# clintpgeorge/LDAGroupedGibbsSampler

Measured on AMD Instinct MI355X. Metric: M tokens sampled/sec (whole node) per Gibbs sweep at K=100, higher is better.
Workload: dtype f64

## Files before the change

ldagroupedgibbssampler_amd/csrc/ggs_api.hip:

```cpp
#include <hip/hip_runtime.h>

#include <algorithm>
#include <cmath>
#include <cstdio>
#include <cstdlib>
#include <cstring>
#include <new>
#include <string>
#include <vector>

#include "ggs_kernels.hpp"
#include "ggs_z_sliced.hpp"
#include "ggs_z_stream.hpp"
#include "ggs_exact_sum.hpp"
#include "ggs_z_pcgs.hpp"
#include "ggs_z_pcgs_wave.hpp"
#include "ggs_z_collapsed.hpp"
#include "ggs_phi_poisson.hpp"
#include "ggs_alias.hpp"
#include "ggs_z_spalias.hpp"
#include "ggs_z_polyaurn_sparse.hpp"
#include "ggs_phi_vs.hpp"
#include "ggs_z_lightpc.hpp"
#include "ggs_z_lightcollapsed.hpp"
// ... 97 lines not shown
  bool have_corpus = false, have_phi = false, in_sweep = false;
  int32_t num_cus = 0;
  LaunchPlan plan;
  const LaunchPlan::ZCfg *cfg = nullptr;
  int32_t *d_chunk_doc1 = nullptr;
  double margin_scale = 1.0;
  double margin_scale32 = 1.0;

  hipStream_t stream = nullptr;
  int64_t *d_doc_ptr = nullptr, *d_chunk_start = nullptr;
  int32_t *d_tok = nullptr, *d_z = nullptr, *d_chunk_doc = nullptr, *d_chunk_len = nullptr;
  int32_t *d_ct_tok = nullptr, *d_ct_idx = nullptr, *d_ct_ip = nullptr, *d_c_docs = nullptr, *d_hot_words = nullptr;
  int64_t Cs = 0, Cc = 0;
  int32_t *d_order = nullptr;
  int64_t pcgs_order_len = 0;
  bool pcgs_wave = false;
  KernelLaunch pcgs_z;
  int64_t pcgs_items = 0;
  int32_t pa_L = 0;
  double pa_t00 = 0;
  double *d_pa_table = nullptr;
  unsigned long long *d_pa_acc = nullptr;
  bool alias_stale = true;
  double *d_alias_ps = nullptr, *d_alias_tn = nullptr;
  int32_t *d_alias_a = nullptr;
  int32_t sp_cap = 0;
  bool have_priors = false;
  int32_t pr_pitch = 0;
  std::vector<uint32_t> pr_mask;
  uint32_t *d_pr_mask = nullptr;
  double *d_pr_sum_phi = nullptr;
  double *d_pr_pref = nullptr, *d_pr_fn = nullptr;
  double alpha_sum = 0;
  unsigned long long *d_mh = nullptr;
  int32_t *d_tpt = nullptr;
  uint16_t *d_nzw = nullptr;
  int32_t *d_nw = nullptr;
  unsigned long long *d_ps_stats = nullptr;
  double vs_pi = 0.5;
  bool vs_global = false;
  int32_t vs_W = 0, vs_pitch = 0;
  uint32_t *d_vs_cz = nullptr, *d_vs_pz = nullptr, *d_vs_und = nullptr;
  uint32_t *d_vs_mask = nullptr;
  int32_t *d_vs_work = nullptr, *d_vs_s_end = nullptr, *d_vs_rounds = nullptr;
  unsigned long long *d_vs_zero = nullptr;
  enum class VsLists { empty, drawn, nonzero } vs_lists = VsLists::empty;
  bool vs_drawn = false;
  uint64_t *d_lcg = nullptr;
  bool lcg_ready = false;
  int32_t num_hot = 0;
  int32_t *d_perm = nullptr, *d_inv_perm = nullptr, *d_zw = nullptr, *d_seg_word = nullptr, *d_seg_begin = nullptr;
  double *d_theta_next = nullptr;
  hipStream_t side = nullptr;
  hipStream_t side_hot = nullptr;
  hipEvent_t ev_hot_fork = nullptr, ev_hot_join = nullptr;
  bool theta_main = true, chain_on_side = false, theta_main_always = false;
  bool whole_sweep = false;
  hipEvent_t hot_fork_from = nullptr;
  hipEvent_t ev_chain_done = nullptr;
  bool z_split = true, z_split_tried = false;
  int32_t warm_tiers = 0, num_warm = 0, warm_rows_max = 0;
  int64_t Cw = 0, warm_chunks_max = 0;
  int32_t *d_wt_pack = nullptr, *d_w_docs = nullptr, *d_warm_words = nullptr;
  int32_t *d_ht_pack = nullptr, *d_h_docs = nullptr;
  int64_t *d_warm_meta = nullptr;
  bool overlap_theta = true;
// ... 615 lines not shown
  return GGS_OK;
}

int launch_phi(ggs_handle *h, bool initial, bool accumulate_mean, Events *E = nullptr) {
  int rc;
  if (h->xg) {
    if ((rc = phi_step_a(h)) || (rc = phi_step_a_clear(h))) return rc;
    if (E) HIP_TRY(h, hipEventRecord(E->x[0], h->stream));
    if ((rc = phi_step_b1(h, initial)) || (rc = phi_step_g0(h)) || (rc = phi_step_b2(h, initial))) return rc;
    if (E) HIP_TRY(h, hipEventRecord(E->x[1], h->stream));
    if ((rc = phi_join_halves(h)) || (rc = phi_step_g1(h))) return rc;
    if (E) HIP_TRY(h, hipEventRecord(E->x[2], h->stream));
    if ((rc = phi_step_c(h, initial, accumulate_mean))) return rc;
    return launch_alias_build(h);
  }
  if (conditional_phi(h, initial) && (rc = launch_sum_phi(h))) return rc;
  if ((rc = launch_phi_slice(h, initial, h->d_n_wk, h->K, h->K, 0, h->d_phiT, h->Kp, h->d_mag, h->d_tot, h->d_n_k, accumulate_mean ? h->d_phi_mean : nullptr)))
    return rc;
  h->n_k_valid = true;
  h->have_phi = true;
  if (h->scheme == Scheme::nzvsspalias) { h->vs_lists = initial ? ggs_handle::VsLists::empty : ggs_handle::VsLists::drawn; if (initial) h->vs_drawn = false; }
  if (h->have_priors && initial && (rc = phi_apply_priors(h))) return rc;
  return launch_alias_build(h);
}

int launch_theta(ggs_handle *h, hipStream_t stream, double *dst, int32_t iteration, int64_t d0 = 0, int64_t d1 = -1, int32_t lds = 0, int32_t docs_per_block = 0) {
  if (d1 < 0) d1 = h->D;
  if (d1 <= d0) return GGS_OK;
  if (docs_per_block <= 0) docs_per_block = h->cfg->theta_docs;
  ThetaParams tp{};
  tp.doc_ptr = h->d_doc_ptr + d0; tp.z = h->d_z; tp.alpha = h->d_alpha; tp.theta = dst + (size_t)d0 * h->K; tp.status = h->d_status;
  tp.num_docs = d1 - d0; tp.doc_base = h->doc_base + d0; tp.seed = h->seed; tp.iteration = (uint32_t)iteration;
  tp.K = h->K; tp.docs_per_block = docs_per_block; tp.queue_cap = std::min(kGammaQueue, h->gamma_queue_cap);
  const int64_t grid = (d1 - d0 + docs_per_block - 1) / docs_per_block;
  void *args[] = {&tp};
  HIP_TRY(h, hipLaunchKernel(h->plan.theta.fn, dim3((unsigned)grid), dim3(kThetaBlock), args, (size_t)(lds ? lds : h->cfg->theta_lds), stream));
  return GGS_OK;
}

#define GGS_KMAX_SWITCH(KERNEL)                                                                                                     \
  switch ((K + 7) / 8) {                                                                                                            \
    case 1: return reinterpret_cast<const void *>(KERNEL<8>);      case 2: return reinterpret_cast<const void *>(KERNEL<16>);       \
    case 3: return reinterpret_cast<const void *>(KERNEL<24>);     case 4: return reinterpret_cast<const void *>(KERNEL<32>);       \
    case 5: return reinterpret_cast<const void *>(KERNEL<40>);     case 6: return reinterpret_cast<const void *>(KERNEL<48>);       \
    case 7: return reinterpret_cast<const void *>(KERNEL<56>);     case 8: return reinterpret_cast<const void *>(KERNEL<64>);       \
    case 9: return reinterpret_cast<const void *>(KERNEL<72>);     case 10: return reinterpret_cast<const void *>(KERNEL<80>);      \
    case 11: return reinterpret_cast<const void *>(KERNEL<88>);    case 12: return reinterpret_cast<const void *>(KERNEL<96>);      \
    case 13: return reinterpret_cast<const void *>(KERNEL<104>);   case 14: return reinterpret_cast<const void *>(KERNEL<112>);     \
    case 15: return reinterpret_cast<const void *>(KERNEL<120>);   case 16: return reinterpret_cast<const void *>(KERNEL<128>);     \
    case 17: return reinterpret_cast<const void *>(KERNEL<136>);   case 18: return reinterpret_cast<const void *>(KERNEL<144>);     \
    case 19: return reinterpret_cast<const void *>(KERNEL<152>);   case 20: return reinterpret_cast<const void *>(KERNEL<160>);     \
    case 21: return reinterpret_cast<const void *>(KERNEL<168>);   case 22: return reinterpret_cast<const void *>(KERNEL<176>);     \
    case 23: return reinterpret_cast<const void *>(KERNEL<184>);   default: return reinterpret_cast<const void *>(KERNEL<192>);     \
  }
const void *sliced_kernel_for(int K) { GGS_KMAX_SWITCH(z_sliced_kernel) }
const void *sliced32_kernel_for(int K) { GGS_KMAX_SWITCH(z_sliced32_kernel) }

const void *hot_kernel_for(int K) { GGS_KMAX_SWITCH(z_hot_kernel) }
const void *warm_kernel_for(int K) { GGS_KMAX_SWITCH(z_warm_kernel) }
const void *pcgs_kernel_for(int K) { GGS_KMAX_SWITCH(pcgs_sliced_kernel) }
const void *polyaurn_kernel_for(int K) { GGS_KMAX_SWITCH(polyaurn_sliced_kernel) }
const void *collapsed_kernel_for(int K) {
  switch ((K + 7) / 8) {
#define GGS_CK(N) case N: return reinterpret_cast<const void *>(pcgs_sliced_kernel<8 * N, true>);
    GGS_CK(1) GGS_CK(2) GGS_CK(3) GGS_CK(4) GGS_CK(5) GGS_CK(6) GGS_CK(7) GGS_CK(8) GGS_CK(9) GGS_CK(10) GGS_CK(11) GGS_CK(12)
    GGS_CK(13) GGS_CK(14) GGS_CK(15) GGS_CK(16) GGS_CK(17) GGS_CK(18) GGS_CK(19) GGS_CK(20) GGS_CK(21) GGS_CK(22) GGS_CK(23)
// ... 54 lines not shown
      pl.z.lds = two_pass ? z_stream_lds_bytes(K) : z_stream1_lds_bytes(K, group, pl.two_rows, regck);
      if (pl.z.lds > kMaxLdsBytes) return GGS_ERR_UNSUPPORTED;
    } else if (sliced) {
      pl.f32 = !kn.phi64.is(1);
      pl.Kp32 = round_up(K, kSlice32Topics);
      pl.ring_base = sliced_ring_base(K); pl.wave_lds = sliced_wave_lds(K); pl.hot_pitch = table_row_pitch(K);
      pl.hot_wave_lds = hot_wave_lds(K); pl.warm_wave_lds = warm_wave_lds(K);
      if (kn.split.set) { pl.split = kn.split.v != 0; pl.split_forced = kn.split.v == 2; }
      pl.hot_cap = pl.split ? table_rows_beside_cold(K, pl.hot_wave_lds) : table_rows_fused(K);
      if (kn.hot.set) pl.hot_cap = std::max(0, std::min(pl.hot_cap, kn.hot.v));
      pl.cold = {pl.f32 ? sliced32_kernel_for(K) : sliced_kernel_for(K), kSlicedWaves * 64, sliced_cold_lds(K), 1};
      pl.hot = {hot_kernel_for(K), kSlicedWaves * 64, table_lds(K, pl.hot_wave_lds, 0), 1};
      pl.warm = {warm_kernel_for(K), kSlicedWaves * 64, table_lds(K, pl.warm_wave_lds, 0), 1};
      pl.warm_docs = warm_docs_for(sliced_kmax(K));
      pl.warm_cap = table_rows_beside_cold(K, pl.warm_wave_lds);
      if (pl.warm_cap < 16) pl.warm_cap = 0;
      if (kn.warm.set) pl.warm_tiers_max = std::max(0, std::min(kWarmMaxTiers, kn.warm.v));
      if (kn.warm_rows.set) pl.warm_cap = std::max(0, std::min(pl.warm_cap, kn.warm_rows.v));
      if (kn.warm_fill.set) pl.warm_min_fill_pct = std::max(1, std::min(100, kn.warm_fill.v));
      if (kn.warm_cpw.set) pl.warm_min_chunks_per_wave = std::max(0, kn.warm_cpw.v);
    } else {
      int T = z_tile_rows_in(kMaxLdsBytes / 6 / kLdsGranule * kLdsGranule, Kp, pitch16);
      if (kn.tile.set) T = kn.tile.v;
      pl.tile_tokens = std::max(8, std::min(64, T));
      pl.z.fn = tile_kernel_for(K);
      pl.z.lds = z_tile_lds_bytes(Kp, pitch16, pl.tile_tokens);
      if (pl.z.lds > kMaxLdsBytes) return GGS_ERR_UNSUPPORTED;
    }
    if (!sliced) {
      pl.z.per_cu = lds_workgroups_per_cu(pl.z.lds, 8);
      if (kn.wpc.set) pl.z.per_cu = std::max(1, kn.wpc.v);
    }
  }
  int B = 64;
  while (B > 1 && theta_lds_bytes(K, B) > 32 * 1024) B >>= 1;
  if (theta_lds_bytes(K, B) > kMaxLdsBytes) return GGS_ERR_UNSUPPORTED;
  pl.theta.fn = reinterpret_cast<const void *>(theta_kernel<kThetaBlock>); pl.theta.block = kThetaBlock;
  const int theta_quarter = (kMaxLdsBytes - 24 * 1024) / 4;
  pl.cfg_plain = {1, pl.z.per_cu, B, std::max(theta_lds_bytes(K, B), theta_quarter), 0};
  pl.theta_docs_main = kn.theta_b.set ? std::max(1, std::min(B, kn.theta_b.v)) : std::min(B, 16);
  pl.theta_lds_main = std::max(theta_lds_bytes(K, pl.theta_docs_main), (kMaxLdsBytes - 24 * 1024) / (kn.theta_wgs.set ? std::max(1, kn.theta_wgs.v) : 5));
  pl.cfg_parts = pl.cfg_plain;
  if (scheme == Scheme::ggs) {
    pl.parts_forced = kn.zparts.set;
    int parts = kn.zparts.set ? std::max(1, std::min(8, kn.zparts.v)) : pl.kernel == 2 ? 8 : 1;
    if (parts > 1 && pl.kernel == 2) {
      const int kBeside = kn.beside.set ? std::max(1, kn.beside.v) : 4;
      int Bt = 64;
      while (Bt > 1 && theta_lds_bytes(K, Bt) > 10 * 1024) Bt >>= 1;
      const int t_lds = theta_lds_bytes(K, Bt), z_alloc = lds_alloc_of(pl.z.lds);
      const int zw = std::min(pl.z.per_cu, (kMaxLdsBytes - kLdsGranule - kBeside * lds_alloc_of(t_lds)) / z_alloc);
      if (t_lds <= 12 * 1024 && zw >= 2)
        pl.cfg_parts = {parts, zw, Bt, std::max(t_lds, theta_quarter), std::max(t_lds, (kMaxLdsBytes - kLdsGranule - zw * z_alloc) / kBeside / kLdsGranule * kLdsGranule)};
      else
        parts = 1;
    }
    pl.cfg_parts.parts = parts;
    return GGS_OK;
  }

  const bool collapsed = scheme == Scheme::collapsed, polyaurn = scheme == Scheme::polyaurn;
  if (K <= kPcgsWaveMaxTopics) {
    const int nb = pcgs_wave_blocks(Kp);
    pl.wave.fn = pcgs_wave_kernel_for(nb, collapsed, polyaurn);
    pl.wave.lds = pcgs_wave_lds_bytes(nb);
    int by_regs = 0;
    if (hipOccupancyMaxActiveBlocksPerMultiprocessor(&by_regs, pl.wave.fn, 64, (size_t)pl.wave.lds) != hipSuccess || by_regs < 1) by_regs = 1;
    pl.wave.per_cu = lds_workgroups_per_cu(pl.wave.lds, std::min(by_regs, 32));
  }
  pl.wave_forced = kn.pcgs_wave.set ? kn.pcgs_wave.v != 0 : K > (collapsed ? kCollapsedWaveFromTopics : polyaurn ? kPolyaurnWaveFromTopics : kPcgsWaveFromTopics);
  if (pl.wave_forced && !pl.wave.fn) return GGS_ERR_UNSUPPORTED;
  const bool lane_sliced = K <= kSlicedMaxTopics && !(kn.pcgs_stream.set && kn.pcgs_stream.v != 0);
  pl.lane.lds = lane_sliced ? pcgs_sliced_lds_bytes(K) : pcgs_z_lds_bytes(K);
  if (pl.lane.lds > kMaxLdsBytes && !pl.wave_forced) return GGS_ERR_UNSUPPORTED;
  pl.lane.per_cu = lds_workgroups_per_cu(pl.lane.lds, 8);
  if (!pl.wave_forced) pl.lane.fn = pcgs_lane_kernel_for(K, lane_sliced, collapsed, polyaurn);
  if (collapsed) pl.serial.fn = reinterpret_cast<const void *>(collapsed_serial_kernel);
  if (has_alias(scheme)) {
    pl.alias_wpb = alias_words_per_block(K);
    pl.alias = {reinterpret_cast<const void *>(alias_build_kernel), 64, (int)alias_lds_bytes(K, pl.alias_wpb), 0};
    pl.alias.per_cu = lds_workgroups_per_cu(pl.alias.lds, 16);
  }
  if (scheme == Scheme::spalias) pl.spalias.fn = reinterpret_cast<const void *>(spalias_wave_kernel);
  if (scheme == Scheme::polyaurn_sparse) {
    pl.wordlist = {reinterpret_cast<const void *>(word_list_build_kernel), kWordListBlock, 0, 8};
// ... 500 lines not shown

}

extern "C" {

int ggs_abi_version(void) { return GGS_ABI_VERSION; }

const char *ggs_last_error(const ggs_handle *h) { return h ? h->err.c_str() : "null handle"; }

int ggs_create(const ggs_config *cfg, ggs_handle **out) {
  if (!cfg || !out) return GGS_ERR_BAD_ARG;
  *out = nullptr;
  if (cfg->struct_size != (int32_t)sizeof(ggs_config)) return GGS_ERR_BAD_ARG;
  if (cfg->num_topics <= 0 || cfg->num_types <= 0 || !(cfg->beta > 0)) return GGS_ERR_BAD_ARG;
  Scheme scheme = Scheme::ggs; int32_t poisson_L = 0;
  if (const int rc = scheme_of(cfg, scheme, poisson_L)) return rc;
  int ndev = 0;
  if (hipGetDeviceCount(&ndev) != hipSuccess || ndev <= 0 || cfg->device_id < 0 || cfg->device_id >= ndev) return GGS_ERR_HIP;
  ggs_handle *h = new (std::nothrow) ggs_handle();
  if (!h) return GGS_ERR_HIP;
  const Knobs kn;
  h->K = cfg->num_topics; h->V = cfg->num_types; h->device = cfg->device_id;
  h->Ks = h->Ksm = h->K; h->k0 = 0;
  h->Kp = (h->K + 1) & ~1;
  h->pitch16 = (h->Kp / 2) | 1;
  h->beta = cfg->beta; h->seed = cfg->seed; h->flags = cfg->flags;
  h->scheme = scheme; h->pa_L = poisson_L;
  h->phi_burn_in = cfg->phi_burn_in; h->phi_thin = cfg->phi_mean_thin > 0 ? cfg->phi_mean_thin : 1;
  h->alpha.assign(h->K, cfg->alpha_scalar);
  if (cfg->alpha) std::copy(cfg->alpha, cfg->alpha + h->K, h->alpha.begin());
  for (double a : h->alpha)
    if (!(a > 0)) { delete h; return GGS_ERR_BAD_ARG; }
  for (double a : h->alpha) h->alpha_sum = h->alpha_sum + a;
  if (kn.margin.set) { h->margin_scale = std::max(1.0, kn.margin.f); h->margin_scale32 = std::max(0.0, kn.margin.f); }
  if (kn.chain.set) h->exact_sum = kn.chain.v == 0;
  if (kn.guided.set) h->sum_guided = kn.guided.v != 0;
  if (kn.no_overlap.set) h->overlap_theta = kn.no_overlap.v == 0;
  if (kn.theta_main.set) { h->theta_main = kn.theta_main.v != 0; h->theta_main_always = kn.theta_main.v == 2; }
  if (kn.gamma_queue.set) h->gamma_queue_cap = std::max(0, kn.gamma_queue.v);
  h->sum_nseg = (h->V + kSumSegRows - 1) / kSumSegRows;

  int rc = GGS_OK;
  auto bail = [&](int code) { ggs_destroy(h); return code; };
  if (hipSetDevice(h->device) != hipSuccess) return bail(GGS_ERR_HIP);
  {
    hipDeviceProp_t prop;
    if (hipGetDeviceProperties(&prop, h->device) != hipSuccess) return bail(GGS_ERR_HIP);
    h->num_cus = prop.multiProcessorCount > 0 ? prop.multiProcessorCount : 256;
    if (kn.num_cus.set) h->num_cus = std::max(1, std::min(h->num_cus, kn.num_cus.v));
  }
  if ((rc = plan_launches(h->K, h->V, h->scheme, kn, h->plan))) return bail(rc);
  h->cfg = &h->plan.cfg_parts;
  h->z_split = h->plan.split;
  if (pcgs_family(h->scheme)) h->pcgs_z = pcgs_entry(h->plan, h->scheme, h->plan.wave_forced);
  for (const KernelLaunch *l : h->plan.all())
    if (l->fn && hipFuncSetAttribute(l->fn, hipFuncAttributeMaxDynamicSharedMemorySize, kMaxLdsBytes) != hipSuccess) return bail(GGS_ERR_HIP);
  for (const void *f : {reinterpret_cast<const void *>(ll_docs_kernel), reinterpret_cast<const void *>(lp_docs_kernel)})
    if (hipFuncSetAttribute(f, hipFuncAttributeMaxDynamicSharedMemorySize, kMaxLdsBytes) != hipSuccess) return bail(GGS_ERR_HIP);
  const bool with_phi = h->scheme != Scheme::lightcollapsed;
  const size_t kv = (size_t)h->K * h->V, phi_elems = (size_t)h->V * h->Kp + kPhiTailPadBytes / 8;
  if ((rc = dev_alloc(h, &h->d_alpha, h->K)) || (with_phi && (rc = dev_alloc(h, &h->d_phiT, phi_elems))) ||
      (rc = dev_alloc(h, &h->d_mag, h->K)) || (rc = dev_alloc(h, &h->d_tot, h->K)) || (rc = dev_alloc(h, &h->d_n_wk, kv)) ||
      (rc = dev_alloc(h, &h->d_n_k, h->K)) || (rc = dev_alloc(h, &h->d_status, 4)))
    return bail(rc);
  if ((h->flags & GGS_FLAG_SAVE_PHI_MEAN) && (rc = dev_alloc(h, &h->d_phi_mean, kv))) return bail(rc);
  if (h->plan.sliced() && h->plan.f32) {
// ... 1366 lines not shown
```

ldagroupedgibbssampler_amd/csrc/ggs_device_math.hpp:

```cpp
#pragma once
#include <hip/hip_runtime.h>
#include <stdint.h>

#include "../../include/ggs_hip.h"
#include "ggs_layout.hpp"

namespace ggs {

struct U4 { uint32_t x, y, z, w; };

__device__ __forceinline__ U4 philox4x32_10(uint32_t c0, uint32_t c1, uint32_t c2, uint32_t c3,
                                            uint32_t k0, uint32_t k1) {
  constexpr uint32_t M0 = 0xD2511F53u, M1 = 0xCD9E8D57u, W0 = 0x9E3779B9u, W1 = 0xBB67AE85u;
#pragma unroll
  for (int r = 0; r < 10; ++r) {
    const uint64_t p0 = (uint64_t)M0 * c0, p1 = (uint64_t)M1 * c2;
    const uint32_t hi0 = (uint32_t)(p0 >> 32), lo0 = (uint32_t)p0;
    const uint32_t hi1 = (uint32_t)(p1 >> 32), lo1 = (uint32_t)p1;
    const uint32_t n0 = hi1 ^ c1 ^ k0, n2 = hi0 ^ c3 ^ k1;
    c0 = n0; c1 = lo1; c2 = n2; c3 = lo0;
    k0 += W0; k1 += W1;
  }
  return U4{c0, c1, c2, c3};
}
// ... 256 lines not shown
      : k0((uint32_t)seed), k1((uint32_t)(seed >> 32)), c0((uint32_t)elem), c1((uint32_t)(elem >> 32)),
        c2base(purpose << 24), c3(iter), pos(0), cached(-1), d0(0), d1(0), next_gauss(0),
        have_gauss(false), exhausted(false) {}

  __device__ __forceinline__ double next_double() {
    const uint32_t blk = pos >> 1;
    if (blk >= (uint32_t)GGS_MAX_BLOCKS) { exhausted = true; return 0.5; }
    if ((int32_t)blk != cached) {
      const U4 o = philox4x32_10(c0, c1, c2base | blk, c3, k0, k1);
      d0 = u53(o.x, o.y);
      d1 = u53(o.z, o.w);
      cached = (int32_t)blk;
    }
    const double d = (pos & 1u) ? d1 : d0;
    ++pos;
    return d;
  }
  __device__ __forceinline__ double next_gaussian() {
    if (have_gauss) { have_gauss = false; return next_gauss; }
    double v1, v2, s;
    do {
      v1 = 2 * next_double() - 1;
      v2 = 2 * next_double() - 1;
      s = v1 * v1 + v2 * v2;
      if (exhausted) return 0.0;
    } while (s >= 1 || s == 0);
    const double multiplier = sqrt(-2 * strict_log(s) / s);
    next_gauss = v2 * multiplier;
    have_gauss = true;
    return v1 * multiplier;
  }
};

__device__ __forceinline__ double prgamma(DrawStream &r, double alpha) {
  const double d = alpha - (1.0 / 3.0);
  const double c = 1.0 / sqrt(9.0 * d);
  for (;;) {
    double x, v;
    do {
      x = r.next_gaussian();
      v = 1.0 + c * x;
      if (r.exhausted) return __builtin_nan("");
    } while (v <= 0.0);
    v = v * v * v;
    const double u = r.next_double();
    if (u < (1.0 - 0.0331 * (x * x) * (x * x))) return d * v;
    if (strict_log(u) < (0.5 * x * x + d * (1.0 - v + strict_log(v)))) return d * v;
    if (r.exhausted) return __builtin_nan("");
  }
}
__device__ __forceinline__ double rgamma(DrawStream &r, double alpha) {
  const bool boost = alpha < 1;
  const double u = r.next_double();
  const double g = prgamma(r, boost ? 1 + alpha : alpha);
  return boost ? g * strict_pow(u, 1.0 / alpha) : g;
}

__device__ __forceinline__ bool rgamma_first_try(uint64_t seed, uint32_t iter, uint32_t purpose, uint64_t elem, double alpha, double &g) {
  const uint32_t k0 = (uint32_t)seed, k1 = (uint32_t)(seed >> 32), c0 = (uint32_t)elem, c1 = (uint32_t)(elem >> 32), c2 = purpose << 24;
  const U4 b0 = philox4x32_10(c0, c1, c2, iter, k0, k1), b1 = philox4x32_10(c0, c1, c2 | 1u, iter, k0, k1),
           b2 = philox4x32_10(c0, c1, c2 | 2u, iter, k0, k1);
  const double u0 = u53(b0.x, b0.y);
  const double a1 = 2 * u53(b0.z, b0.w) - 1, a2 = 2 * u53(b1.x, b1.y) - 1, sa = a1 * a1 + a2 * a2;
  const double w = u53(b1.z, b1.w);
  const double e1 = 2 * w - 1, e2 = 2 * u53(b2.x, b2.y) - 1, sb = e1 * e1 + e2 * e2;
  const bool ok_a = !(sa >= 1 || sa == 0), ok_b = !(sb >= 1 || sb == 0);
  if (!(ok_a || ok_b)) return false;
  const double v1 = ok_a ? a1 : e1, s = ok_a ? sa : sb;
  const double u = ok_a ? w : u53(b2.z, b2.w);
  const double multiplier = sqrt(-2 * strict_log(s) / s);
  const double x = v1 * multiplier;
  const bool boost = alpha < 1;
  const double shape = boost ? 1 + alpha : alpha;
  const double d = shape - (1.0 / 3.0);
  const double c = 1.0 / sqrt(9.0 * d);
  double v = 1.0 + c * x;
  if (!(v > 0.0)) return false;
  v = v * v * v;
  if (!(u < (1.0 - 0.0331 * (x * x) * (x * x)))) return false;
  const double r = d * v;
  g = boost ? r * strict_pow(u0, 1.0 / alpha) : r;
  return true;
}

}
```

ldagroupedgibbssampler_amd/csrc/ggs_kernels.hpp:

```cpp
#pragma once
#include "ggs_device_math.hpp"
#include "ggs_exact_sum.hpp"

namespace ggs {

constexpr double kJavaMinValue = 4.9e-324;

__device__ __forceinline__ uint32_t udiv_magic(uint32_t d) { return d > 1 ? (uint32_t)((0x100000000ull + d - 1) / d) : 0u; }
__device__ __forceinline__ int udiv_small(int x, uint32_t m) { return m ? (int)__umulhi((uint32_t)x, m) : x; }

enum StatusBits : uint32_t {
  ST_NEGATIVE_COUNT = 1u << 0,
  ST_INVALID_TOPIC = 1u << 1,
  ST_RNG_EXHAUSTED = 1u << 2,
  ST_BAD_SHAPE = 1u << 3,
  ST_INVARIANT = 1u << 4,
};

struct ThetaParams {
  const int64_t *doc_ptr;
  const int32_t *z;
  const double *alpha;
  double *theta;
  uint32_t *status;
  int64_t num_docs, doc_base;
  uint64_t seed;
  uint32_t iteration;
  int32_t K, docs_per_block;
  int32_t queue_cap;
};

constexpr int kGammaQueue = 768;
constexpr int kThetaQueueBytes = 8 + 2 * kGammaQueue;
constexpr int theta_lds_bytes(const int K, const int b) { return (int)((size_t)K * (b | 1) * 8 + (size_t)b * 20 + kThetaQueueBytes); }

template <int BLOCK>
__global__ __launch_bounds__(BLOCK) void theta_kernel(ThetaParams p) {
  extern __shared__ __align__(16) unsigned char smem[];
  const int K = p.K, B = p.docs_per_block, BP = B | 1;
  double *gam = reinterpret_cast<double *>(smem);
  int32_t *hist = reinterpret_cast<int32_t *>(smem);
  double *mag = gam + (size_t)K * BP;
  double *tot = mag + B;
  int32_t *len = reinterpret_cast<int32_t *>(tot + B);
  int32_t *qn = len + B;
  uint16_t *queue = reinterpret_cast<uint16_t *>(qn + 2);

  const int tid = threadIdx.x;
  const int64_t d0 = (int64_t)blockIdx.x * B;
  const int nb = (int)min((int64_t)B, p.num_docs - d0);

  for (int i = tid; i < K * BP; i += BLOCK) hist[2 * i] = 0;
  if (tid == 0) *qn = 0;
  __syncthreads();

  constexpr int NW = BLOCK / 64;
  const int wave = tid >> 6, lane = tid & 63;
  for (int b = wave; b < nb; b += NW) {
    const int64_t beg = p.doc_ptr[d0 + b], end = p.doc_ptr[d0 + b + 1];
    if (lane == 0) len[b] = (int32_t)(end - beg);
    for (int64_t i = beg + lane; i < end; i += 64) atomicAdd(&hist[2 * (p.z[i] * BP + b)], 1);
  }
  __syncthreads();

  if (tid < nb && len[tid] > 0) {
    double m = 0;
    for (int k = 0; k < K; ++k) m += (double)hist[2 * (k * BP + tid)] + p.alpha[k];
    mag[tid] = m;
  }
  __syncthreads();

  auto shape_of = [&](int k, int b) {
    const double pk = (double)hist[2 * (k * BP + b)] + p.alpha[k];
    const double m = mag[b];
    return (pk / m) * m;
  };
  auto draw_general = [&](int k, int b, double shape) {
    DrawStream rs(p.seed, p.iteration, GGS_PURPOSE_THETA, (uint64_t)(p.doc_base + d0 + b) * (uint64_t)K + (uint64_t)k);
    const double g = rgamma(rs, shape);
    if (rs.exhausted) atomicOr(p.status, ST_RNG_EXHAUSTED);
    return g;
  };
  const uint32_t m_nb = udiv_magic((uint32_t)max(nb, 1)), m_K = udiv_magic((uint32_t)K);
  for (int i = tid; i < nb * K; i += BLOCK) {
    const int k = udiv_small(i, m_nb), b = i - k * nb;
    if (len[b] == 0) continue;
    const double shape = shape_of(k, b);
    double g;
    if (shape > 0) {
      if (!rgamma_first_try(p.seed, p.iteration, GGS_PURPOSE_THETA, (uint64_t)(p.doc_base + d0 + b) * (uint64_t)K + (uint64_t)k, shape, g)) {
        const int slot = atomicAdd(qn, 1);
        if (slot < p.queue_cap) { queue[slot] = (uint16_t)i; continue; }
        g = draw_general(k, b, shape);
      }
    } else {
      g = __builtin_nan("");
      atomicOr(p.status, ST_BAD_SHAPE);
    }
    gam[k * BP + b] = g;
  }
  __syncthreads();
  for (int q = tid, m = min(*qn, p.queue_cap); q < m; q += BLOCK) {
    const int i = queue[q], k = udiv_small(i, m_nb), b = i - k * nb;
    gam[k * BP + b] = draw_general(k, b, shape_of(k, b));
  }
  __syncthreads();

  if (tid < nb && len[tid] > 0) {
    double s = 0;
    for (int k = 0; k < K; ++k) s += gam[k * BP + tid];
    tot[tid] = s;
  }
  __syncthreads();

  for (int i = tid; i < nb * K; i += BLOCK) {
    const int b = udiv_small(i, m_K), k = i - b * K;
    if (len[b] == 0) continue;
    double v = gam[k * BP + b];
    const double s = tot[b];
    if (s != 0) {
      v = v / s;
      if (v <= 0) v = kJavaMinValue;
    }
// ... 214 lines not shown

struct PhiGammaParams {
  const int32_t *n_wk;
  const double *mag;
  double *phiT;
  uint32_t *status;
  uint64_t seed;
  uint32_t iteration, purpose;
  int32_t K, Kp, V;
  int32_t cnt_pitch, k0;
  double beta;
  double prior_pm;
  int32_t initial;
  int32_t kc, ncg;
  int32_t seg_begin, seg_end;
  int32_t queue_cap;
  int32_t prio;
  const double *guess;
  double *fn;
  const uint32_t *zero_mask;
  int32_t mask_pitch;
  int32_t undrawn_negative;
};
constexpr double kConditionalMinGamma = 0.0001;

constexpr int kPhiCols = 6, kPhiQueue = 128;

enum PhiDraw { kDrawPlain, kDrawPriors, kDrawVS };
template <int MODE>
__device__ __forceinline__ void phi_gamma_body(const PhiGammaParams &p) {
  constexpr bool PRIORS = MODE == kDrawPriors, MASKED = MODE != kDrawPlain;
  if (p.prio) __builtin_amdgcn_s_setprio(1);
  __shared__ uint16_t queue[kPhiQueue];
  __shared__ int32_t qn;
  __shared__ double acc_lo[kPhiCols], acc_hi[kPhiCols];
  __shared__ int32_t e_los[kPhiCols], aheads[kPhiCols], flag_s[kPhiCols];
  const int lane = threadIdx.x;
  const int64_t tiles = (int64_t)(p.seg_end - p.seg_begin) * p.ncg;
  auto shape_of = [&](int v, int k) {
    const int32_t cnt = p.n_wk[(size_t)v * p.cnt_pitch + k];
    if (p.initial) return (cnt == 0) ? p.prior_pm : p.prior_pm + (double)cnt;
    const double pk = p.beta + (double)cnt;
    if constexpr (MODE == kDrawVS) return pk;
    const double m = p.mag[k];
    return (pk / m) * m;
  };
  auto draw_general = [&](int v, int k, double shape) {
    DrawStream rs(p.seed, p.iteration, p.purpose, (uint64_t)(p.k0 + k) * (uint64_t)p.V + (uint64_t)v);
    const double g = rgamma(rs, shape);
    if (rs.exhausted) atomicOr(p.status, ST_RNG_EXHAUSTED);
    return g;
  };
  const uint32_t m_ncg = udiv_magic((uint32_t)p.ncg);
  for (int64_t tile = blockIdx.x; tile < tiles; tile += gridDim.x) {
    const int si = udiv_small((int)tile, m_ncg), cg = (int)tile - si * p.ncg;
    const int seg = p.seg_begin + si, v0 = seg * 64, kb = cg * p.kc, kw = min(p.kc, p.K - kb);
    const int rows = min(64, p.V - v0), n = rows * kw;
    const uint32_t m_kw = udiv_magic((uint32_t)kw);
    __syncthreads();
    if (lane < kw) {
      SegCand c{kSegNoGuess, true};
      if (p.guess) c = seg_candidates(p.guess[(size_t)seg * p.K + kb + lane], p.guess[(size_t)(seg + 1) * p.K + kb + lane]);
      e_los[lane] = c.e_lo; aheads[lane] = c.ahead ? 1 : 0; acc_lo[lane] = 0; acc_hi[lane] = 0; flag_s[lane] = 0;
    }
    if (lane == 0) qn = 0;
    __syncthreads();
    auto emit = [&](int v, int c, double g) {
      if constexpr (PRIORS) { if (g <= 0) g = kConditionalMinGamma; }
      p.phiT[(size_t)v * p.Kp + kb + c] = g;
      const int e_lo = e_los[c];
      if (e_lo == kSegNoGuess) return;
      double q_lo, q_hi;
      int fl;
      seg_quantise(g, e_lo, q_lo, q_hi, fl);
      seg_accumulate(&acc_lo[c], &acc_hi[c], &flag_s[c], q_lo, q_hi, fl);
    };
#pragma unroll 1
    for (int j = lane; j < n; j += 64) {
      const int dv = udiv_small(j, m_kw), v = v0 + dv, c = j - dv * kw, k = kb + c;
      if constexpr (MASKED) {
        const int kg = p.k0 + k;
        if ((p.zero_mask[(size_t)v * p.mask_pitch + (kg >> 5)] >> (kg & 31)) & 1u) {
          p.phiT[(size_t)v * p.Kp + k] = (MODE == kDrawVS && p.undrawn_negative) ? -0.0 : 0.0;
          continue;
        }
      }
      const double shape = shape_of(v, k);
      double g;
      if (shape > 0) {
        if (!rgamma_first_try(p.seed, p.iteration, p.purpose, (uint64_t)(p.k0 + k) * (uint64_t)p.V + (uint64_t)v, shape, g)) {
          const int slot = atomicAdd(&qn, 1);
          if (slot < p.queue_cap) { queue[slot] = (uint16_t)j; continue; }
          g = draw_general(v, k, shape);
        }
      } else {
        g = __builtin_nan("");
        atomicOr(p.status, ST_BAD_SHAPE);
      }
      emit(v, c, g);
    }
    __syncthreads();
    for (int q = lane, m = min(qn, p.queue_cap); q < m; q += 64) {
      const int j = queue[q], dv = udiv_small(j, m_kw), v = v0 + dv, c = j - dv * kw;
      emit(v, c, draw_general(v, kb + c, shape_of(v, kb + c)));
    }
    __syncthreads();
    if (p.guess && lane < kw)
      seg_compose(SegCand{e_los[lane], aheads[lane] != 0}, acc_lo[lane], acc_hi[lane], flag_s[lane], 0.0, p.fn + ((size_t)seg * p.K + kb + lane) * 4);
  }
}
template <bool PRIORS>
__global__ __launch_bounds__(64) void phi_gamma_kernel(PhiGammaParams p) { phi_gamma_body<PRIORS ? kDrawPriors : kDrawPlain>(p); }
__global__ __launch_bounds__(64) void phi_gamma_vs_kernel(PhiGammaParams p) { phi_gamma_body<kDrawVS>(p); }

__device__ __forceinline__ float phi32_of(const double x) { return (x >= 0.0 && x <= 1.0) ? (float)x : __builtin_nanf(""); }

enum PhiNorm { kPhiDirichlet, kPhiPolyaurn, kPhiConditional, kPhiVS };
template <int MODE>
__device__ __forceinline__ void phi_normalise_body(double *phiT, const double *tot, int32_t K, int32_t Kp, int32_t V, double *phi_mean, float *phiT32,
                                                   int32_t Kp32, const double *sum_phi = nullptr) {
  __builtin_amdgcn_s_setprio(3);
  const int64_t n = (int64_t)V * K;
  const int64_t stride = (int64_t)gridDim.x * blockDim.x;
// ... 199 lines not shown
```

Measured before the change: 16480.

## Precompute gamma constants for zero-count cells and sort cells into table/general lists

Splits the Marsaglia-Tsang gamma setup (d, c, 1/alpha) into a reusable GammaConsts struct. In the theta and phi kernels, cells with zero counts (and symmetric alpha for theta) share one shape per doc or column, so their constants are computed once and kept in LDS. Cells are partitioned by wave ballots into a table list and a general list, so whole waves use the precomputed constants and skip per-cell sqrt and divide. This costs an extra pre-pass over the counts, more LDS (the theta block sizing is adjusted to fit it), and a branch on list membership.

```diff
diff --git a/ldagroupedgibbssampler_amd/csrc/ggs_api.hip b/ldagroupedgibbssampler_amd/csrc/ggs_api.hip
--- a/ldagroupedgibbssampler_amd/csrc/ggs_api.hip
+++ b/ldagroupedgibbssampler_amd/csrc/ggs_api.hip
@@ -153,6 +153,7 @@
   double *d_pr_sum_phi = nullptr;
   double *d_pr_pref = nullptr, *d_pr_fn = nullptr;
   double alpha_sum = 0;
+  bool alpha_symmetric = false;
   unsigned long long *d_mh = nullptr;
   int32_t *d_tpt = nullptr;
   uint16_t *d_nzw = nullptr;
@@ -834,6 +835,7 @@
   tp.doc_ptr = h->d_doc_ptr + d0; tp.z = h->d_z; tp.alpha = h->d_alpha; tp.theta = dst + (size_t)d0 * h->K; tp.status = h->d_status;
   tp.num_docs = d1 - d0; tp.doc_base = h->doc_base + d0; tp.seed = h->seed; tp.iteration = (uint32_t)iteration;
   tp.K = h->K; tp.docs_per_block = docs_per_block; tp.queue_cap = std::min(kGammaQueue, h->gamma_queue_cap);
+  tp.sym_alpha = h->alpha_symmetric ? 1 : 0;
   const int64_t grid = (d1 - d0 + docs_per_block - 1) / docs_per_block;
   void *args[] = {&tp};
   HIP_TRY(h, hipLaunchKernel(h->plan.theta.fn, dim3((unsigned)grid), dim3(kThetaBlock), args, (size_t)(lds ? lds : h->cfg->theta_lds), stream));
@@ -954,11 +956,11 @@
       if (kn.wpc.set) pl.z.per_cu = std::max(1, kn.wpc.v);
     }
   }
+  const int theta_quarter = (kMaxLdsBytes - 24 * 1024) / 4;
   int B = 64;
-  while (B > 1 && theta_lds_bytes(K, B) > 32 * 1024) B >>= 1;
+  while (B > 1 && (theta_cells_lds_bytes(K, B) > 32 * 1024 || (B > 16 && theta_lds_bytes(K, B) > theta_quarter))) B >>= 1;
   if (theta_lds_bytes(K, B) > kMaxLdsBytes) return GGS_ERR_UNSUPPORTED;
   pl.theta.fn = reinterpret_cast<const void *>(theta_kernel<kThetaBlock>); pl.theta.block = kThetaBlock;
-  const int theta_quarter = (kMaxLdsBytes - 24 * 1024) / 4;
   pl.cfg_plain = {1, pl.z.per_cu, B, std::max(theta_lds_bytes(K, B), theta_quarter), 0};
   pl.theta_docs_main = kn.theta_b.set ? std::max(1, std::min(B, kn.theta_b.v)) : std::min(B, 16);
   pl.theta_lds_main = std::max(theta_lds_bytes(K, pl.theta_docs_main), (kMaxLdsBytes - 24 * 1024) / (kn.theta_wgs.set ? std::max(1, kn.theta_wgs.v) : 5));
@@ -968,11 +970,13 @@
     int parts = kn.zparts.set ? std::max(1, std::min(8, kn.zparts.v)) : pl.kernel == 2 ? 8 : 1;
     if (parts > 1 && pl.kernel == 2) {
       const int kBeside = kn.beside.set ? std::max(1, kn.beside.v) : 4;
+      const int z_alloc = lds_alloc_of(pl.z.lds);
+      auto z_waves_beside = [&](int theta_lds) { return std::min(pl.z.per_cu, (kMaxLdsBytes - kLdsGranule - kBeside * lds_alloc_of(theta_lds)) / z_alloc); };
       int Bt = 64;
-      while (Bt > 1 && theta_lds_bytes(K, Bt) > 10 * 1024) Bt >>= 1;
-      const int t_lds = theta_lds_bytes(K, Bt), z_alloc = lds_alloc_of(pl.z.lds);
-      const int zw = std::min(pl.z.per_cu, (kMaxLdsBytes - kLdsGranule - kBeside * lds_alloc_of(t_lds)) / z_alloc);
-      if (t_lds <= 12 * 1024 && zw >= 2)
+      while (Bt > 1 && theta_cells_lds_bytes(K, Bt) > 10 * 1024) Bt >>= 1;
+      const int zw = z_waves_beside(theta_cells_lds_bytes(K, Bt));
+      const int t_lds = theta_lds_bytes(K, Bt);
+      if (theta_cells_lds_bytes(K, Bt) <= 12 * 1024 && zw >= 2)
         pl.cfg_parts = {parts, zw, Bt, std::max(t_lds, theta_quarter), std::max(t_lds, (kMaxLdsBytes - kLdsGranule - zw * z_alloc) / kBeside / kLdsGranule * kLdsGranule)};
       else
         parts = 1;
@@ -1539,6 +1543,7 @@
   for (double a : h->alpha)
     if (!(a > 0)) { delete h; return GGS_ERR_BAD_ARG; }
   for (double a : h->alpha) h->alpha_sum = h->alpha_sum + a;
+  h->alpha_symmetric = std::all_of(h->alpha.begin(), h->alpha.end(), [&](double a) { return std::memcmp(&a, &h->alpha[0], sizeof a) == 0; });
   if (kn.margin.set) { h->margin_scale = std::max(1.0, kn.margin.f); h->margin_scale32 = std::max(0.0, kn.margin.f); }
   if (kn.chain.set) h->exact_sum = kn.chain.v == 0;
   if (kn.guided.set) h->sum_guided = kn.guided.v != 0;
diff --git a/ldagroupedgibbssampler_amd/csrc/ggs_device_math.hpp b/ldagroupedgibbssampler_amd/csrc/ggs_device_math.hpp
--- a/ldagroupedgibbssampler_amd/csrc/ggs_device_math.hpp
+++ b/ldagroupedgibbssampler_amd/csrc/ggs_device_math.hpp
@@ -312,9 +312,24 @@
   }
 };
 
-__device__ __forceinline__ double prgamma(DrawStream &r, double alpha) {
-  const double d = alpha - (1.0 / 3.0);
-  const double c = 1.0 / sqrt(9.0 * d);
+struct GammaConsts {
+  double shape;
+  double d, c;
+  double inv_alpha;
+  bool boost;
+};
+__device__ __forceinline__ GammaConsts gamma_consts(double alpha) {
+  GammaConsts k;
+  k.shape = alpha;
+  k.boost = alpha < 1;
+  const double shape = k.boost ? 1 + alpha : alpha;
+  k.d = shape - (1.0 / 3.0);
+  k.c = 1.0 / sqrt(9.0 * k.d);
+  k.inv_alpha = k.boost ? 1.0 / alpha : 0.0;
+  return k;
+}
+
+__device__ __forceinline__ double prgamma(DrawStream &r, const double d, const double c) {
   for (;;) {
     double x, v;
     do {
@@ -329,14 +344,14 @@
     if (r.exhausted) return __builtin_nan("");
   }
 }
-__device__ __forceinline__ double rgamma(DrawStream &r, double alpha) {
-  const bool boost = alpha < 1;
+__device__ __forceinline__ double rgamma(DrawStream &r, const GammaConsts &k) {
   const double u = r.next_double();
-  const double g = prgamma(r, boost ? 1 + alpha : alpha);
-  return boost ? g * strict_pow(u, 1.0 / alpha) : g;
-}
-
-__device__ __forceinline__ bool rgamma_first_try(uint64_t seed, uint32_t iter, uint32_t purpose, uint64_t elem, double alpha, double &g) {
+  const double g = prgamma(r, k.d, k.c);
+  return k.boost ? g * strict_pow(u, k.inv_alpha) : g;
+}
+__device__ __forceinline__ double rgamma(DrawStream &r, double alpha) { return rgamma(r, gamma_consts(alpha)); }
+
+__device__ __forceinline__ bool rgamma_first_try(uint64_t seed, uint32_t iter, uint32_t purpose, uint64_t elem, const GammaConsts &k, double &g) {
   const uint32_t k0 = (uint32_t)seed, k1 = (uint32_t)(seed >> 32), c0 = (uint32_t)elem, c1 = (uint32_t)(elem >> 32), c2 = purpose << 24;
   const U4 b0 = philox4x32_10(c0, c1, c2, iter, k0, k1), b1 = philox4x32_10(c0, c1, c2 | 1u, iter, k0, k1),
            b2 = philox4x32_10(c0, c1, c2 | 2u, iter, k0, k1);
@@ -350,17 +365,16 @@
   const double u = ok_a ? w : u53(b2.z, b2.w);
   const double multiplier = sqrt(-2 * strict_log(s) / s);
   const double x = v1 * multiplier;
-  const bool boost = alpha < 1;
-  const double shape = boost ? 1 + alpha : alpha;
-  const double d = shape - (1.0 / 3.0);
-  const double c = 1.0 / sqrt(9.0 * d);
-  double v = 1.0 + c * x;
+  double v = 1.0 + k.c * x;
   if (!(v > 0.0)) return false;
   v = v * v * v;
   if (!(u < (1.0 - 0.0331 * (x * x) * (x * x)))) return false;
-  const double r = d * v;
-  g = boost ? r * strict_pow(u0, 1.0 / alpha) : r;
+  const double r = k.d * v;
+  g = k.boost ? r * strict_pow(u0, k.inv_alpha) : r;
   return true;
 }
-
-}
+__device__ __forceinline__ bool rgamma_first_try(uint64_t seed, uint32_t iter, uint32_t purpose, uint64_t elem, double alpha, double &g) {
+  return rgamma_first_try(seed, iter, purpose, elem, gamma_consts(alpha), g);
+}
+
+}
diff --git a/ldagroupedgibbssampler_amd/csrc/ggs_kernels.hpp b/ldagroupedgibbssampler_amd/csrc/ggs_kernels.hpp
--- a/ldagroupedgibbssampler_amd/csrc/ggs_kernels.hpp
+++ b/ldagroupedgibbssampler_amd/csrc/ggs_kernels.hpp
@@ -28,11 +28,13 @@
   uint32_t iteration;
   int32_t K, docs_per_block;
   int32_t queue_cap;
+  int32_t sym_alpha;
 };
 
 constexpr int kGammaQueue = 768;
 constexpr int kThetaQueueBytes = 8 + 2 * kGammaQueue;
-constexpr int theta_lds_bytes(const int K, const int b) { return (int)((size_t)K * (b | 1) * 8 + (size_t)b * 20 + kThetaQueueBytes); }
+constexpr int theta_cells_lds_bytes(const int K, const int b) { return (int)((size_t)K * (b | 1) * 8 + (size_t)b * 20 + kThetaQueueBytes); }
+constexpr int theta_lds_bytes(const int K, const int b) { return theta_cells_lds_bytes(K, b) + (int)((size_t)b * sizeof(GammaConsts) + (size_t)K * b * 2); }
 
 template <int BLOCK>
 __global__ __launch_bounds__(BLOCK) void theta_kernel(ThetaParams p) {
@@ -42,16 +44,18 @@
   int32_t *hist = reinterpret_cast<int32_t *>(smem);
   double *mag = gam + (size_t)K * BP;
   double *tot = mag + B;
-  int32_t *len = reinterpret_cast<int32_t *>(tot + B);
+  GammaConsts *ctab = reinterpret_cast<GammaConsts *>(tot + B);
+  int32_t *len = reinterpret_cast<int32_t *>(ctab + B);
   int32_t *qn = len + B;
   uint16_t *queue = reinterpret_cast<uint16_t *>(qn + 2);
+  uint16_t *list = queue + kGammaQueue;
 
   const int tid = threadIdx.x;
   const int64_t d0 = (int64_t)blockIdx.x * B;
   const int nb = (int)min((int64_t)B, p.num_docs - d0);
 
   for (int i = tid; i < K * BP; i += BLOCK) hist[2 * i] = 0;
-  if (tid == 0) *qn = 0;
+  if (tid < 2) qn[tid] = 0;
   __syncthreads();
 
   constexpr int NW = BLOCK / 64;
@@ -67,8 +71,30 @@
     double m = 0;
     for (int k = 0; k < K; ++k) m += (double)hist[2 * (k * BP + tid)] + p.alpha[k];
     mag[tid] = m;
-  }
-  __syncthreads();
+    const double pk = (double)0 + p.alpha[0];
+    ctab[tid] = gamma_consts((pk / m) * m);
+  }
+  const uint32_t m_nb = udiv_magic((uint32_t)max(nb, 1)), m_K = udiv_magic((uint32_t)K);
+  const int ncell = nb * K;
+  for (int i0 = wave * 64; i0 < ncell; i0 += BLOCK) {
+    const int i = i0 + lane;
+    bool listed = false, a = false;
+    if (i < ncell) {
+      const int k = udiv_small(i, m_nb), b = i - k * nb;
+      listed = len[b] > 0;
+      a = listed && p.sym_alpha && hist[2 * (k * BP + b)] == 0;
+    }
+    const unsigned long long ma = __ballot(a), mb = __ballot(listed && !a);
+    uint32_t base = 0;
+    if (lane == 0) base = atomicAdd(reinterpret_cast<uint32_t *>(qn + 1), (uint32_t)__popcll(ma) | (uint32_t)__popcll(mb) << 16);
+    base = (uint32_t)__shfl((int)base, 0);
+    const unsigned long long mine = a ? ma : mb;
+    const int rank = (int)__builtin_amdgcn_mbcnt_hi((uint32_t)(mine >> 32), __builtin_amdgcn_mbcnt_lo((uint32_t)mine, 0u));
+    if (a) list[(int)(base & 0xffffu) + rank] = (uint16_t)i;
+    else if (listed) list[ncell - 1 - ((int)(base >> 16) + rank)] = (uint16_t)i;
+  }
+  __syncthreads();
+  const int n_a = (int)((uint32_t)qn[1] & 0xffffu), n_b = (int)((uint32_t)qn[1] >> 16);
 
   auto shape_of = [&](int k, int b) {
     const double pk = (double)hist[2 * (k * BP + b)] + p.alpha[k];
@@ -81,14 +107,17 @@
     if (rs.exhausted) atomicOr(p.status, ST_RNG_EXHAUSTED);
     return g;
   };
-  const uint32_t m_nb = udiv_magic((uint32_t)max(nb, 1)), m_K = udiv_magic((uint32_t)K);
-  for (int i = tid; i < nb * K; i += BLOCK) {
+  for (int pos = tid; pos < n_a + n_b; pos += BLOCK) {
+    const int i = list[pos < n_a ? pos : ncell - n_b + (pos - n_a)];
     const int k = udiv_small(i, m_nb), b = i - k * nb;
-    if (len[b] == 0) continue;
-    const double shape = shape_of(k, b);
+    const bool table = __ballot(pos >= n_a) == 0;
+    const double shape = table ? ctab[b].shape : shape_of(k, b);
     double g;
     if (shape > 0) {
-      if (!rgamma_first_try(p.seed, p.iteration, GGS_PURPOSE_THETA, (uint64_t)(p.doc_base + d0 + b) * (uint64_t)K + (uint64_t)k, shape, g)) {
+      const uint64_t elem = (uint64_t)(p.doc_base + d0 + b) * (uint64_t)K + (uint64_t)k;
+      const bool drawn = table ? rgamma_first_try(p.seed, p.iteration, GGS_PURPOSE_THETA, elem, ctab[b], g)
+                               : rgamma_first_try(p.seed, p.iteration, GGS_PURPOSE_THETA, elem, shape, g);
+      if (!drawn) {
         const int slot = atomicAdd(qn, 1);
         if (slot < p.queue_cap) { queue[slot] = (uint16_t)i; continue; }
         g = draw_general(k, b, shape);
@@ -369,19 +398,21 @@
   constexpr bool PRIORS = MODE == kDrawPriors, MASKED = MODE != kDrawPlain;
   if (p.prio) __builtin_amdgcn_s_setprio(1);
   __shared__ uint16_t queue[kPhiQueue];
+  __shared__ uint16_t list[64 * kPhiCols];
+  __shared__ GammaConsts ctab[kPhiCols];
   __shared__ int32_t qn;
   __shared__ double acc_lo[kPhiCols], acc_hi[kPhiCols];
   __shared__ int32_t e_los[kPhiCols], aheads[kPhiCols], flag_s[kPhiCols];
   const int lane = threadIdx.x;
   const int64_t tiles = (int64_t)(p.seg_end - p.seg_begin) * p.ncg;
-  auto shape_of = [&](int v, int k) {
-    const int32_t cnt = p.n_wk[(size_t)v * p.cnt_pitch + k];
+  auto shape_of_count = [&](int32_t cnt, int k) {
     if (p.initial) return (cnt == 0) ? p.prior_pm : p.prior_pm + (double)cnt;
     const double pk = p.beta + (double)cnt;
     if constexpr (MODE == kDrawVS) return pk;
     const double m = p.mag[k];
     return (pk / m) * m;
   };
+  auto shape_of = [&](int v, int k) { return shape_of_count(p.n_wk[(size_t)v * p.cnt_pitch + k], k); };
   auto draw_general = [&](int v, int k, double shape) {
     DrawStream rs(p.seed, p.iteration, p.purpose, (uint64_t)(p.k0 + k) * (uint64_t)p.V + (uint64_t)v);
     const double g = rgamma(rs, shape);
@@ -399,8 +430,32 @@
       SegCand c{kSegNoGuess, true};
       if (p.guess) c = seg_candidates(p.guess[(size_t)seg * p.K + kb + lane], p.guess[(size_t)(seg + 1) * p.K + kb + lane]);
       e_los[lane] = c.e_lo; aheads[lane] = c.ahead ? 1 : 0; acc_lo[lane] = 0; acc_hi[lane] = 0; flag_s[lane] = 0;
+      ctab[lane] = gamma_consts(shape_of_count(0, kb + lane));
     }
     if (lane == 0) qn = 0;
+    int n_a = 0, n_b = 0;
+#pragma unroll 1
+    for (int j0 = 0; j0 < n; j0 += 64) {
+      const int j = j0 + lane;
+      bool listed = false, a = false;
+      if (j < n) {
+        const int dv = udiv_small(j, m_kw), v = v0 + dv, k = kb + (j - dv * kw);
+        listed = true;
+        if constexpr (MASKED) {
+          const int kg = p.k0 + k;
+          if ((p.zero_mask[(size_t)v * p.mask_pitch + (kg >> 5)] >> (kg & 31)) & 1u) {
+            p.phiT[(size_t)v * p.Kp + k] = (MODE == kDrawVS && p.undrawn_negative) ? -0.0 : 0.0;
+            listed = false;
+          }
+        }
+        a = listed && p.n_wk[(size_t)v * p.cnt_pitch + k] == 0;
+      }
+      const unsigned long long ma = __ballot(a), mb = __ballot(listed && !a), mine = a ? ma : mb;
+      const int rank = (int)__builtin_amdgcn_mbcnt_hi((uint32_t)(mine >> 32), __builtin_amdgcn_mbcnt_lo((uint32_t)mine, 0u));
+      if (a) list[n_a + rank] = (uint16_t)j;
+      else if (listed) list[n - 1 - (n_b + rank)] = (uint16_t)j;
+      n_a += (int)__popcll(ma); n_b += (int)__popcll(mb);
+    }
     __syncthreads();
     auto emit = [&](int v, int c, double g) {
       if constexpr (PRIORS) { if (g <= 0) g = kConditionalMinGamma; }
@@ -413,19 +468,17 @@
       seg_accumulate(&acc_lo[c], &acc_hi[c], &flag_s[c], q_lo, q_hi, fl);
     };
 #pragma unroll 1
-    for (int j = lane; j < n; j += 64) {
+    for (int pos = lane; pos < n_a + n_b; pos += 64) {
+      const int j = list[pos < n_a ? pos : n - n_b + (pos - n_a)];
       const int dv = udiv_small(j, m_kw), v = v0 + dv, c = j - dv * kw, k = kb + c;
-      if constexpr (MASKED) {
-        const int kg = p.k0 + k;
-        if ((p.zero_mask[(size_t)v * p.mask_pitch + (kg >> 5)] >> (kg & 31)) & 1u) {
-          p.phiT[(size_t)v * p.Kp + k] = (MODE == kDrawVS && p.undrawn_negative) ? -0.0 : 0.0;
-          continue;
-        }
-      }
-      const double shape = shape_of(v, k);
+      const bool table = __ballot(pos >= n_a) == 0;
+      const double shape = table ? ctab[c].shape : shape_of(v, k);
       double g;
       if (shape > 0) {
-        if (!rgamma_first_try(p.seed, p.iteration, p.purpose, (uint64_t)(p.k0 + k) * (uint64_t)p.V + (uint64_t)v, shape, g)) {
+        const uint64_t elem = (uint64_t)(p.k0 + k) * (uint64_t)p.V + (uint64_t)v;
+        const bool drawn = table ? rgamma_first_try(p.seed, p.iteration, p.purpose, elem, ctab[c], g)
+                                 : rgamma_first_try(p.seed, p.iteration, p.purpose, elem, shape, g);
+        if (!drawn) {
           const int slot = atomicAdd(&qn, 1);
           if (slot < p.queue_cap) { queue[slot] = (uint16_t)j; continue; }
           g = draw_general(v, k, shape);
```

After: 16980 (median of 6 runs). 3.1% higher.
